# aligirayhanozbay/poisson_CNN

Measured on AMD Instinct MI355X. Metric: grids/sec (fwd+bwd) at 1024^2, higher is better.
Workload: dtype f32; 1 GPU; c4: Homogeneous_Poisson_NN_Legacy(hpnn.json) full train step (fwd+bwd+loss+Adam), 8 x 1024x1024 Dirichlet grids per GPU; global_batch=8, parallelism=dp1, math=fp32, ranks_seen=1

## Files before the change

include/pcnn.h:

```cpp
#ifndef PCNN_H
#define PCNN_H
#include <stddef.h>
#include <stdint.h>
#ifdef __cplusplus
extern "C" {
#endif

typedef struct pcnn_handle_s* pcnn_handle;

enum { PCNN_PAD_CONSTANT = 0, PCNN_PAD_SYMMETRIC = 1, PCNN_PAD_REFLECT = 2 };
enum { PCNN_ACT_LINEAR = 0, PCNN_ACT_LEAKY_RELU = 1, PCNN_ACT_TANH = 2, PCNN_ACT_RELU = 3 };
enum { PCNN_POOL_AVERAGE = 0, PCNN_POOL_MAX = 1 };
enum { PCNN_RESIZE_NEAREST = 0, PCNN_RESIZE_BILINEAR = 1, PCNN_RESIZE_BICUBIC = 2,
       PCNN_RESIZE_BICUBIC_LEGACY_ALIGN_CORNERS = 3  };

int pcnn_create(int device, void* hip_stream, pcnn_handle* out);
int pcnn_destroy(pcnn_handle h);
int pcnn_set_stream(pcnn_handle h, void* hip_stream);
int pcnn_sync(pcnn_handle h);
const char* pcnn_last_error(pcnn_handle h);
int pcnn_version(void);
uint32_t pcnn_crc32c(const void* data, size_t n, uint32_t crc);

#define PCNN_UNIQUE_ID_BYTES 128
// ... 52 lines not shown
                     const float* w1, const float* b1, const float* w2, const float* b2, float* o0, float* a1, float* o1, float* y);

int pcnn_conv2d_bwd_spectral_eligible(pcnn_handle h, const pcnn_conv_desc* d, const pcnn_conv_desc* dg);
int pcnn_conv2d_bwd_spectral(pcnn_handle h, const pcnn_conv_desc* d, const pcnn_conv_desc* dg, const float* x, const float* dz, const float* w_flipped,
                             const float* residual, float* dx, float* dw);
typedef struct pcnn_post_desc {
  const float* act_out; int ld_act_out; int act; float act_alpha;
  float* dbias; float* raw_out; int ld_raw;
} pcnn_post_desc;
int pcnn_conv2d_bwd_spectral_post_eligible(pcnn_handle h, const pcnn_conv_desc* d, const pcnn_conv_desc* dg);
int pcnn_conv2d_bwd_spectral_post(pcnn_handle h, const pcnn_conv_desc* d, const pcnn_conv_desc* dg, const float* x, const float* dz, const float* w_flipped,
                                  const float* residual, float* dx, float* dw, const pcnn_post_desc* post);

int pcnn_conv2d_dgrad_post_eligible(pcnn_handle h, const pcnn_conv_desc* dg, const float* dz, const float* residual, const float* dx, const pcnn_post_desc* post);
int pcnn_conv2d_dgrad_post(pcnn_handle h, const pcnn_conv_desc* dg, const float* dz, const float* w_flipped, const float* residual, float* dx,
                           const pcnn_post_desc* post);

int pcnn_debug_forward_spectrum32(pcnn_handle h, int H, int W, int C, const float* x, int Vy, int Vx, int oy, int ox, int pad_mode, float pad_value,
                                  int ylim, int xlim, int pack, float* out, size_t out_floats);
int pcnn_debug_tile_spectrum64(pcnn_handle h, int H, int W, int C, const float* x, int ylim, int xlim, float* out);

size_t pcnn_colsum_workspace(int C);
int pcnn_conv2d_epilogue_bwd(pcnn_handle h, int64_t npix, int C, const float* dy, int lddy, const float* a, int lda,
                             const float* bn_scale, int act, float act_alpha, float* dz, int lddz,
                             float* dbias, float* dsum_dy_a, float* dsum_dy, void* workspace, size_t workspace_bytes);
int pcnn_conv2d_epilogue_bwd_absmax(pcnn_handle h, int64_t npix, int C, const float* dy, int lddy, const float* a, int lda,
                                    const float* bn_scale, int act, float act_alpha, float* dz, int lddz, float* dbias,
                                    float* dsum_dy_a, float* dsum_dy, float* dz_absmax, void* workspace, size_t workspace_bytes);

int pcnn_pad_fold_bwd(pcnn_handle h, int N, int H, int W, int C, int pt, int pb, int pl, int pr, int pad_mode,
                      const float* gp, int ldgp, float* gx, int ldgx, int accumulate);
int pcnn_pad_fold_bwd_post_eligible(int C, int ldgp, int ld_add, const void* gp, const void* add_to, const pcnn_post_desc* post, int lddz, const void* dz);
int pcnn_pad_fold_bwd_post(pcnn_handle h, int N, int H, int W, int C, int pt, int pb, int pl, int pr, int pad_mode, const float* gp, int ldgp,
                           const float* add_to, int ld_add, const pcnn_post_desc* post, const float* bn_scale, float* dsum_dy_a, float* dsum_dy,
                           float* dz, int lddz, void* workspace, size_t workspace_bytes);

int pcnn_bn_fold(pcnn_handle h, int n, const float* gamma, const float* beta, const float* mean, const float* var, float eps,
                 float* scale, float* shift);
int pcnn_bn_fold_bwd(pcnn_handle h, int n, const float* s_dy_a, const float* s_dy, const float* mean, const float* var, float eps,
                     float* dgamma, float* dbeta);

int pcnn_channel_affine(pcnn_handle h, int64_t npix, int C, const float* x, int ldx, const float* scale, const float* shift,
                        const float* residual, int ld_res, float* y, int ldy);
int pcnn_bn_train_fwd(pcnn_handle h, int64_t npix, int C, const float* a, int lda, const float* gamma, const float* beta, float eps,
                      float momentum, float* moving_mean, float* moving_var, float* mean, float* inv_std, float* scale, float* scratch_2C,
                      const float* residual, int ld_res, float* y, int ldy, void* workspace, size_t workspace_bytes);
int pcnn_bn_train_bwd(pcnn_handle h, int64_t npix, int C, const float* dy, int lddy, const float* a, int lda, const float* scale,
                      const float* mean, const float* inv_std, float* dgamma, float* dbeta, float* scratch_4C, float* da, int ldda,
                      void* workspace, size_t workspace_bytes);

int pcnn_pool2d_fwd(pcnn_handle h, int kind, int N, int H, int W, int C, int f, const float* x, int ldx, float* y, int ldy);
int pcnn_pool2d_bwd(pcnn_handle h, int kind, int N, int H, int W, int C, int f, const float* x, int ldx,
                    const float* y, int ldy, const float* dy, int lddy, float* dx, int lddx, int accumulate);

int pcnn_deconv_fwd(pcnn_handle h, int N, int hc, int wc, int Cin, int H, int W, int Cout, int f, const float* x, int ldx,
                    const float* k, const float* bias, float alpha, float beta, float* y, int ldy);
int pcnn_deconv_bwd_data(pcnn_handle h, int N, int hc, int wc, int Cin, int H, int W, int Cout, int f, const float* dy, int lddy,
                         const float* k, float alpha, float* dx, int lddx);
size_t pcnn_deconv_wgrad_workspace(int N, int hc, int wc, int Cin, int Cout, int f);
int pcnn_deconv_bwd_filter(pcnn_handle h, int N, int hc, int wc, int Cin, int H, int W, int Cout, int f, const float* x, int ldx,
                           const float* dy, int lddy, float alpha, float* dk, float* dbias, void* workspace, size_t workspace_bytes);

typedef struct {
  int N, H, W, Cin, ldx;
  int Ho, Wo, Cout, ldy;
  int k;
  int act; float act_alpha;
  float dropout_rate; uint32_t dropout_seed; uint32_t dropout_layer;
  int ld_act_out;
  int accumulate;
} pcnn_wide_desc;
int pcnn_wide_conv2d_fwd(pcnn_handle h, const pcnn_wide_desc* d, const float* x, const float* w, const float* bias, float* y);
int pcnn_wide_conv2d_dgrad(pcnn_handle h, const pcnn_wide_desc* d, const float* dz, const float* wf, const float* act_out, float* dx);
size_t pcnn_wide_conv2d_wgrad_workspace(const pcnn_wide_desc* d);
int pcnn_wide_conv2d_wgrad(pcnn_handle h, const pcnn_wide_desc* d, const float* x, const float* dz, float* dw, float* dbias, void* workspace,
                           size_t workspace_bytes);
int pcnn_wide_deconv_fwd(pcnn_handle h, const pcnn_wide_desc* d, const float* x, const float* k, const float* bias, float* y);
int pcnn_wide_deconv_bwd_data(pcnn_handle h, const pcnn_wide_desc* d, const float* dz, const float* k, const float* act_out, float* dx);
size_t pcnn_wide_deconv_bwd_filter_workspace(const pcnn_wide_desc* d);
int pcnn_wide_deconv_bwd_filter(pcnn_handle h, const pcnn_wide_desc* d, const float* x, const float* dz, float* dk, void* workspace,
                                size_t workspace_bytes);

int pcnn_resize_tables(int method, int n_in, int n_out, int32_t* idx , float* wt );
int pcnn_resize_fwd(pcnn_handle h, int N, int hc, int wc, int C, int Ho, int Wo, const float* x, int ldx,
                    const int32_t* idx_y, const float* wt_y, const int32_t* idx_x, const float* wt_x,
                    float alpha, float beta, float* y, int ldy);
typedef struct pcnn_resize_src {
  const float* x; int hc, wc, ldx;
  const int32_t* idx_y; const float* wt_y; const int32_t* idx_x; const float* wt_x;
} pcnn_resize_src;
int pcnn_resize_fwd_multi_eligible(int N, int C, int Ho, int Wo, int nsrc, const pcnn_resize_src* src, const float* y, int ldy);
int pcnn_resize_fwd_multi(pcnn_handle h, int N, int C, int Ho, int Wo, int nsrc, const pcnn_resize_src* src, float alpha, float beta, float* y, int ldy);
int pcnn_resize_bwd(pcnn_handle h, int N, int hc, int wc, int C, int Ho, int Wo, const float* dy, int lddy,
                    const int32_t* idx_y, const float* wt_y, const int32_t* idx_x, const float* wt_x,
                    float alpha, float* tmp, float* dx, int lddx);

size_t pcnn_grouped_conv2d_wgrad_workspace(const pcnn_conv_desc* d);
int pcnn_grouped_conv2d_uses_mfma(const pcnn_conv_desc* d, int what);
int pcnn_grouped_conv2d_fwd(pcnn_handle h, const pcnn_conv_desc* d, const float* x, const float* w, long long w_sample_stride, const float* bias,
                            long long bias_sample_stride, int flip_transpose, float* y);
int pcnn_grouped_conv2d_wgrad(pcnn_handle h, const pcnn_conv_desc* d, const float* x, const float* dz, float* dw, long long dw_sample_stride, void* workspace);
int pcnn_grouped_bias_grad(pcnn_handle h, int N, long long HW, int C, const float* dz, int lddz, float* dbias, long long bias_sample_stride);
int pcnn_grouped_deconv_fwd(pcnn_handle h, int N, int H, int W, int Cin, int Ho, int Wo, int Cout, int f, const float* x, const float* k,
                            long long k_sample_stride, const float* bias, long long bias_sample_stride, float* y);
int pcnn_grouped_deconv_bwd_data(pcnn_handle h, int N, int H, int W, int Cin, int Ho, int Wo, int Cout, int f, const float* dy, const float* k,
                                 long long k_sample_stride, float* dx);
// ... 191 lines not shown
```

poisson_cnn_amd/csrc/pool_resize.hip:

```cpp
#include <math.h>
#include <vector>
#include "pcnn_internal.h"

namespace {

__device__ __forceinline__ void win(int o, int f, int pb, int n, int& a, int& b) {
  a = o * f - pb; b = a + f;
  if (a < 0) a = 0;
  if (b > n) b = n;
}

__global__ void pool_fwd_small_vec4_kernel(int kind, int N, int H, int W, int C, int f, int Ho, int Wo, int pby, int pbx,
                                           const float* __restrict__ x, int ldx, float* __restrict__ y, int ldy);
__global__ void pool_fwd_small_kernel(int kind, int N, int H, int W, int C, int f, int Ho, int Wo, int pby, int pbx,
                                      const float* __restrict__ x, int ldx, float* __restrict__ y, int ldy) {
  const int64_t total = (int64_t)N * Ho * Wo * C;
  for (int64_t i = (int64_t)blockIdx.x * blockDim.x + threadIdx.x; i < total; i += (int64_t)gridDim.x * blockDim.x) {
    const int c = i % C; int64_t r = i / C; const int ox = r % Wo; r /= Wo; const int oy = r % Ho; const int n = r / Ho;
    int y0, y1, x0, x1;
    win(oy, f, pby, H, y0, y1); win(ox, f, pbx, W, x0, x1);
    float acc = kind == PCNN_POOL_MAX ? -INFINITY : 0.f;
    for (int yy = y0; yy < y1; ++yy)
      for (int xx = x0; xx < x1; ++xx) {
        const float v = x[(((int64_t)n * H + yy) * W + xx) * ldx + c];
// ... 61 lines not shown
    int y0, y1, x0, x1;
    win(oy, f, pby, H, y0, y1); win(ox, f, pbx, W, x0, x1);
    const float cnt = (float)((y1 - y0) * (x1 - x0));
    const float* src = dy + (((int64_t)n * Ho + oy) * Wo + ox) * lddy + c;
    float* dst = dx + (((int64_t)n * H + yy) * W + xx) * lddx + c;
    if (V == 4) {
      const float4 g = *reinterpret_cast<const float4*>(src);
      float4 o = make_float4(g.x / cnt, g.y / cnt, g.z / cnt, g.w / cnt);
      if (accumulate) { const float4 d = *reinterpret_cast<const float4*>(dst); o.x += d.x; o.y += d.y; o.z += d.z; o.w += d.w; }
      *reinterpret_cast<float4*>(dst) = o;
    } else {
      const float g = *src / cnt;
      *dst = accumulate ? *dst + g : g;
    }
  }
}

__global__ void pool_bwd_max_kernel(int N, int H, int W, int C, int f, int Ho, int Wo, int pby, int pbx, const float* __restrict__ x, int ldx,
                                    const float* __restrict__ dy, int lddy, float* __restrict__ dx, int lddx) {
  const int64_t total = (int64_t)N * Ho * Wo * C;
  for (int64_t i = (int64_t)blockIdx.x * blockDim.x + threadIdx.x; i < total; i += (int64_t)gridDim.x * blockDim.x) {
    const int c = i % C; int64_t r = i / C; const int ox = r % Wo; r /= Wo; const int oy = r % Ho; const int n = r / Ho;
    int y0, y1, x0, x1;
    win(oy, f, pby, H, y0, y1); win(ox, f, pbx, W, x0, x1);
    float best = -INFINITY; int by = y0, bx = x0;
    for (int yy = y0; yy < y1; ++yy)
      for (int xx = x0; xx < x1; ++xx) {
        const float v = x[(((int64_t)n * H + yy) * W + xx) * ldx + c];
        if (v > best) { best = v; by = yy; bx = xx; }
      }
    dx[(((int64_t)n * H + by) * W + bx) * lddx + c] += dy[(((int64_t)n * Ho + oy) * Wo + ox) * lddy + c];
  }
}

__global__ void zero_strided_kernel(int64_t npix, int C, float* __restrict__ y, int ldy) {
  const int64_t total = npix * C;
  for (int64_t i = (int64_t)blockIdx.x * blockDim.x + threadIdx.x; i < total; i += (int64_t)gridDim.x * blockDim.x) y[(i / C) * ldy + i % C] = 0.f;
}

template <int V> struct ChanVec;
template <> struct ChanVec<1> {
  float v[1];
  __device__ static ChanVec load(const float* p) { ChanVec r; r.v[0] = *p; return r; }
  __device__ void store(float* p) const { *p = v[0]; }
};
template <> struct ChanVec<4> {
  float v[4];
  __device__ static ChanVec load(const float* p) {
    const float4 t = *reinterpret_cast<const float4*>(p);
    ChanVec r; r.v[0] = t.x; r.v[1] = t.y; r.v[2] = t.z; r.v[3] = t.w; return r;
  }
  __device__ void store(float* p) const { *reinterpret_cast<float4*>(p) = make_float4(v[0], v[1], v[2], v[3]); }
};

template <int V>
__global__ __launch_bounds__(256) void resize_fwd_kernel(int N, int hc, int wc, int C, int Ho, int Wo, const float* __restrict__ x, int ldx,
                                  const int32_t* __restrict__ iy, const float* __restrict__ wy, const int32_t* __restrict__ ix,
                                  const float* __restrict__ wx, float alpha, float beta, float* __restrict__ y, int ldy) {
  const int CV = C / V;
  const int64_t total = (int64_t)N * Ho * Wo * CV;
  for (int64_t i = (int64_t)blockIdx.x * blockDim.x + threadIdx.x; i < total; i += (int64_t)gridDim.x * blockDim.x) {
    const int c = (int)(i % CV) * V; int64_t r = i / CV; const int ox = r % Wo; r /= Wo; const int oy = r % Ho; const int n = r / Ho;
    float wxb[4]; int ixb[4];
#pragma unroll
    for (int b = 0; b < 4; ++b) { wxb[b] = wx[ox * 4 + b]; ixb[b] = ix[ox * 4 + b]; }
    float acc[V];
#pragma unroll
    for (int j = 0; j < V; ++j) acc[j] = 0.f;
#pragma unroll
    for (int a = 0; a < 4; ++a) {
      const float wya = wy[oy * 4 + a];
      if (wya == 0.f) continue;
      const float* row = x + ((int64_t)n * hc + iy[oy * 4 + a]) * wc * ldx + c;
      float t[V];
#pragma unroll
      for (int j = 0; j < V; ++j) t[j] = 0.f;
#pragma unroll
      for (int b = 0; b < 4; ++b) {
        if (wxb[b] != 0.f) {
          const ChanVec<V> q = ChanVec<V>::load(row + (int64_t)ixb[b] * ldx);
#pragma unroll
          for (int j = 0; j < V; ++j) t[j] += wxb[b] * q.v[j];
        }
      }
#pragma unroll
      for (int j = 0; j < V; ++j) acc[j] += wya * t[j];
    }
    float* dst = &y[(((int64_t)n * Ho + oy) * Wo + ox) * ldy + c];
    ChanVec<V> o;
    if (beta == 0.f) {
#pragma unroll
      for (int j = 0; j < V; ++j) o.v[j] = alpha * acc[j];
    } else {
      const ChanVec<V> old = ChanVec<V>::load(dst);
#pragma unroll
      for (int j = 0; j < V; ++j) o.v[j] = beta * old.v[j] + alpha * acc[j];
    }
    o.store(dst);
  }
}

constexpr int RESIZE_RPB = 8;
__global__ __launch_bounds__(256) void resize_fwd_y_kernel(int N, int hc, int C, int Ho, int Wo, const float* __restrict__ t, const int32_t* __restrict__ iy,
                                                           const float* __restrict__ wy, float alpha, float beta, float* __restrict__ y, int ldy) {
  const int CV = C >> 2;
  const int u = blockIdx.x * 256 + threadIdx.x;
// ... 201 lines not shown
}

static bool vec4_ok(int C, const void* a, int lda, const void* b, int ldb) {
  return C % 4 == 0 && lda % 4 == 0 && ldb % 4 == 0 && ((reinterpret_cast<uintptr_t>(a) | reinterpret_cast<uintptr_t>(b)) & 15) == 0;
}

static dim3 grid1d(int64_t total, int block = 256, int maxb = 16384) {
  int64_t b = pcnn_cdiv64(total, block);
  if (b > maxb) b = maxb;
  if (b < 1) b = 1;
  return dim3((unsigned)b);
}
static int pow2_ge(int c) { int p = 1; while (p < c) p <<= 1; return p; }

}

extern "C" int pcnn_pool2d_fwd(pcnn_handle h, int kind, int N, int H, int W, int C, int f, const float* x, int ldx, float* y, int ldy) {
  PCNN_REQUIRE(h, h && x && y && f >= 1 && (kind == 0 || kind == 1), "pcnn_pool2d_fwd: bad argument");
  const int Ho = pcnn_cdiv(H, f), Wo = pcnn_cdiv(W, f), pby = (Ho * f - H) / 2, pbx = (Wo * f - W) / 2;
  if (f * f <= 16 || C > 256) {
    if (vec4_ok(C, x, ldx, y, ldy))
      hipLaunchKernelGGL(pool_fwd_small_vec4_kernel, grid1d((int64_t)N * Ho * Wo * (C / 4)), dim3(256), 0, h->stream, kind, N, H, W, C, f, Ho, Wo, pby, pbx, x, ldx, y, ldy);
    else
      hipLaunchKernelGGL(pool_fwd_small_kernel, grid1d((int64_t)N * Ho * Wo * C), dim3(256), 0, h->stream, kind, N, H, W, C, f, Ho, Wo, pby, pbx, x, ldx, y, ldy);
  } else {
    hipLaunchKernelGGL(pool_fwd_large_kernel, dim3((unsigned)((int64_t)N * Ho * Wo)), dim3(256), 0, h->stream, kind, N, H, W, C, pow2_ge(C), f, Ho,
                       Wo, pby, pbx, x, ldx, y, ldy);
  }
  PCNN_CHECK_LAUNCH(h, "pcnn_pool2d_fwd");
  return 0;
}

extern "C" int pcnn_pool2d_bwd(pcnn_handle h, int kind, int N, int H, int W, int C, int f, const float* x, int ldx, const float* y, int ldy,
                               const float* dy, int lddy, float* dx, int lddx, int accumulate) {
  PCNN_REQUIRE(h, h && dy && dx && f >= 1 && (kind == 0 || kind == 1), "pcnn_pool2d_bwd: bad argument");
  (void)y; (void)ldy;
  const int Ho = pcnn_cdiv(H, f), Wo = pcnn_cdiv(W, f), pby = (Ho * f - H) / 2, pbx = (Wo * f - W) / 2;
  if (kind == PCNN_POOL_AVERAGE) {
    if (vec4_ok(C, dy, lddy, dx, lddx))
      hipLaunchKernelGGL(pool_bwd_avg_kernel<4>, grid1d((int64_t)N * H * W * (C / 4)), dim3(256), 0, h->stream, N, H, W, C, f, Ho, Wo, pby, pbx, dy, lddy, dx,
                         lddx, accumulate);
    else
      hipLaunchKernelGGL(pool_bwd_avg_kernel<1>, grid1d((int64_t)N * H * W * C), dim3(256), 0, h->stream, N, H, W, C, f, Ho, Wo, pby, pbx, dy, lddy, dx, lddx,
                         accumulate);
  } else {
    PCNN_REQUIRE(h, x, "pcnn_pool2d_bwd: max pooling needs the forward input");
    if (!accumulate) {
      hipLaunchKernelGGL(zero_strided_kernel, grid1d((int64_t)N * H * W * C), dim3(256), 0, h->stream, (int64_t)N * H * W, C, dx, lddx);
    }
    hipLaunchKernelGGL(pool_bwd_max_kernel, grid1d((int64_t)N * Ho * Wo * C), dim3(256), 0, h->stream, N, H, W, C, f, Ho, Wo, pby, pbx, x, ldx, dy, lddy, dx,
                       lddx);
  }
  PCNN_CHECK_LAUNCH(h, "pcnn_pool2d_bwd");
  return 0;
}

extern "C" int pcnn_resize_tables(int method, int n_in, int n_out, int32_t* idx, float* wt) {
  if (!idx || !wt || n_in < 1 || n_out < 1) return 1;
  const float scale = (float)n_in / (float)n_out;
  static std::vector<float> table;
  if (method == PCNN_RESIZE_BICUBIC && table.empty()) {
    const float a = -0.5f;
    table.resize((1024 + 1) * 2);
    for (int i = 0; i <= 1024; ++i) {
      float x = (float)i * 1.0f / 1024.0f;
      table[2 * i] = ((a + 2) * x - (a + 3)) * x * x + 1;
      x += 1.0f;
      table[2 * i + 1] = ((a * x - 5 * a) * x + 8 * a) * x - 4 * a;
    }
  }
  for (int o = 0; o < n_out; ++o) {
    int32_t* I = idx + 4 * o; float* Wt = wt + 4 * o;
    for (int k = 0; k < 4; ++k) { I[k] = 0; Wt[k] = 0.f; }
    if (method == PCNN_RESIZE_NEAREST) {
      int i = (int)floorf(((float)o + 0.5f) * scale);
      I[0] = i < 0 ? 0 : (i > n_in - 1 ? n_in - 1 : i); Wt[0] = 1.f;
    } else if (method == PCNN_RESIZE_BILINEAR) {
      const float src = ((float)o + 0.5f) * scale - 0.5f;
      const float fl = floorf(src);
      const int lo = fl > 0.f ? (int)fl : 0;
      const int hi = (int)fminf(ceilf(src), (float)(n_in - 1));
      const float lerp = src - fl;
      I[0] = lo; Wt[0] = 1.0f - lerp; I[1] = hi; Wt[1] = lerp;
    } else if (method == PCNN_RESIZE_BICUBIC) {
      const float src = ((float)o + 0.5f) * scale - 0.5f;
      const int loc = (int)floorf(src);
      const float delta = src - (float)loc;
      const int off = (int)lrintf(delta * 1024.0f);
      float w4[4] = {table[off * 2 + 1], table[off * 2], table[(1024 - off) * 2], table[(1024 - off) * 2 + 1]};
      float sum = 0.f;
      for (int k = 0; k < 4; ++k) {
        const int raw = loc - 1 + k;
        const int cl = raw < 0 ? 0 : (raw > n_in - 1 ? n_in - 1 : raw);
        if (cl != raw) w4[k] = 0.f;
        I[k] = cl; sum += w4[k];
      }
      if (fabsf(sum) >= 1000.0f * 1.17549435e-38f) {
        const float inv = 1.0f / sum;
        for (int k = 0; k < 4; ++k) w4[k] *= inv;
      }
      for (int k = 0; k < 4; ++k) Wt[k] = w4[k];
    } else if (method == PCNN_RESIZE_BICUBIC_LEGACY_ALIGN_CORNERS) {
      static std::vector<float> legacy;
      if (legacy.empty()) {
        const float a = -0.75f;
        legacy.resize((1024 + 1) * 2);
// ... 93 lines not shown
```

poisson_cnn_amd/models.py:

```python
import collections
import copy
import os

import numpy as np
import torch

from . import layers as L
from . import ops
from .utils import BC_EDGES, get_init_arguments_from_config, neumann_flags, neumann_mask, split_indices


def process_normalizations(normalizations):
    types, defaults = ['rhs_max_magnitude'], [False]
    if normalizations is None:
        return dict(zip(types, defaults))
    normalizations = dict(normalizations)
    for k, d in zip(types, defaults):
        normalizations.setdefault(k, d)
    if isinstance(normalizations['rhs_max_magnitude'], bool) and normalizations['rhs_max_magnitude']:
        normalizations['rhs_max_magnitude'] = 1.0
    return normalizations


def process_output_scaling_modes(output_scalings):
# ... 368 lines not shown
            history.update({'val_' + k: [] for k in self._VAL_KEYS})
        self.stop_training = False
        for cb in callbacks:
            cb.set_model(self)
        fetch = _Prefetcher(dataset, self.device)
        try:
            return self._fit_epochs(dataset, epochs, callbacks, verbose, steps_per_epoch, history, fetch, validation)
        finally:
            fetch.close()

    def _fit_epochs(self, dataset, epochs, callbacks, verbose, steps_per_epoch, history, fetch, validation=None):
        for epoch in range(epochs):
            n = steps_per_epoch if steps_per_epoch is not None else len(dataset)
            agg = {'loss': 0.0, 'mse': 0.0}
            logs = {'loss': float('nan'), 'mse': float('nan')}
            step = -1
            if n > 0:
                fetch.request(0)
            for step in range(n):
                inp, tar = fetch.take()
                logs = self.train_step((tuple(inp), tar))
                if step + 1 < n:
                    fetch.request(step + 1)
                logs = _host_logs(logs)
                for k in agg:
                    agg[k] += logs[k]
                for cb in callbacks:
                    cb.on_batch_end(step, logs)
                if self.stop_training:
                    break
            logs = {'loss': logs['loss'], 'mse': logs['mse'], 'lr': self.optimizer.learning_rate,
                    'loss_epoch_mean': agg['loss'] / max(step + 1, 1), 'mse_epoch_mean': agg['mse'] / max(step + 1, 1)}
            val_line = ''
            if validation is not None and (epoch + 1) % validation['freq'] == 0:
                res = self.evaluate(return_dict=True, **{k: v for k, v in validation.items() if k != 'freq'})
                logs.update({'val_' + k: res[k] for k in self._VAL_KEYS})
                val_line = ''.join(' - val_%s: %.6g' % (k, res[k]) for k in self._VAL_KEYS)
            for k in logs:
                history[k].append(logs[k])
            if verbose:
                print('Epoch %d/%d - loss: %.6g - mse: %.6g - lr: %.3g (epoch mean loss %.6g)%s'
                      % (epoch + 1, epochs, logs['loss'], logs['mse'], logs['lr'], logs['loss_epoch_mean'], val_line), flush=True)
            for cb in callbacks:
                cb.on_epoch_end(epoch, logs)
            if hasattr(dataset, 'on_epoch_end'):
                dataset.on_epoch_end()
            if self.stop_training:
                break
        return history


_BRANCH_STREAMS = os.environ.get('PCNN_BRANCH_STREAMS', '1') != '0'

MergePlan = collections.namedtuple('MergePlan', 'pyramid order stream tail')


def merge_plan(branches, H, W, coarse_factor):
    pyramid = {}
    for f in sorted({f for f, down, pool, _ in branches if down == 'pool' and pool in ('average', 'avg') and H % f == 0 and W % f == 0}):
        pyramid[f] = max([g for g in pyramid if f % g == 0], default=None)
    coarse = [i for i, b in enumerate(branches) if b[0] >= coarse_factor]
    order = [i for i in range(len(branches)) if i not in coarse] + coarse
    stream = {i: (k + 1 if branches[i][0] in pyramid else 0) for k, i in enumerate(coarse)}
    ntail = 0
    while ntail < min(3, len(order) - 1) and branches[order[-1 - ntail]][3] is not None:
        ntail += 1
    return MergePlan(pyramid, order, stream, order[len(order) - ntail:] if ntail >= 2 else [])


class _BottleneckMerge:

    def __init__(self, blocks, ctx, filters):
        self.blocks, self.ctx = list(blocks), ctx
        self.branches = [(b.f, b.down_method, b.pool, b.resize_method) for b in self.blocks]
        self.alpha = 1.0 / float(len(self.blocks) * filters)
        self._saved = None

    def pool_pyramid(self, x, plan):
        pyr = {}
        for f, parent in plan.pyramid.items():
            pyr[f] = ops.pool2d_fwd(x if parent is None else pyr[parent], f if parent is None else f // parent, 'average')
        return pyr

    def forward(self, initial, merged, training, coarse_factor):
        H, W = initial.shape[1], initial.shape[2]
        blocks, alpha = self.blocks, self.alpha
        plan = merge_plan(self.branches, H, W, coarse_factor)
        pyr = self.pool_pyramid(initial, plan)
        pending, streams = {}, {}
        if plan.stream and self.ctx.use_side and _BRANCH_STREAMS:
            ready = torch.cuda.Event()
            ready.record(torch.cuda.current_stream())
            for i, k in plan.stream.items():
                st = self.ctx.branch_stream(k)
                with torch.cuda.stream(st):
                    st.wait_event(ready)
                    o = blocks[i].forward_convs(initial, training, pyr.get(blocks[i].f))
                    done = torch.cuda.Event()
                    done.record(st)
                pending[i] = (o, done)
                if training:
                    streams[i] = st
        tail = []
        for n, i in enumerate(plan.order):
            b = blocks[i]
            if i in pending:
                o, done = pending[i]
                torch.cuda.current_stream().wait_event(done)
                o.record_stream(torch.cuda.current_stream())
            else:
                o = b.forward_convs(initial, training, pyr.get(b.f))
            b.note_upsampled(o, training)
            if i in plan.tail:
                tail.append((b, o))
            else:
                b.up_into(o, (H, W), merged, alpha, 0.0 if n == 0 else 1.0)
        if tail and ops.resize_fwd_multi([o for _, o in tail], (H, W), [b.resize_method for b, _ in tail], alpha=alpha, beta=1.0, out=merged) is None:
            for b, o in tail:
                b.up_into(o, (H, W), merged, alpha, 1.0)
        self._saved = (initial, pyr, plan.pyramid, streams) if training else None

    def backward(self, dmerged, d_initial):
        initial, pyr, parents, streams = self._saved
        self._saved = None
        alpha = self.alpha
        grads = {}
        late = []
        main = torch.cuda.current_stream()

        def add(f, g):
            grads[f] = g if f not in grads else ops.axpby(1.0, g, 1.0, grads[f])
        for i, b in enumerate(self.blocks):
            st = streams.get(i)
            if st is None:
                for _, g_prev, done_prev in late:
                    if g_prev is None:
                        main.wait_event(done_prev)
                g = b.backward_from(dmerged, alpha, d_initial)
                if g is not None:
                    add(b.f, g)
                continue
            dco = b.backward_up(dmerged, alpha)
            ev = torch.cuda.Event()
            ev.record(main)
            with torch.cuda.stream(st):
                st.wait_event(ev)
                dco.record_stream(st)
                g = b.backward_convs(dco, d_initial)
                done = torch.cuda.Event()
                done.record(st)
            late.append((b, g, done))
        for b, g, done in late:
            main.wait_event(done)
            if g is not None:
                g.record_stream(main)
                add(b.f, g)
        for f in sorted(grads, reverse=True):
            parent = parents[f]
            if parent is None:
                ops.pool2d_bwd(initial, grads[f], f, 'average', dx=d_initial, accumulate=True)
            else:
                if parent not in grads:
                    grads[parent] = torch.zeros_like(pyr[parent])
                ops.pool2d_bwd(pyr[parent], grads[f], f // parent, 'average', dx=grads[parent], accumulate=True)


class Homogeneous_Poisson_NN_Legacy(_ModelBase):
    model_name = 'Homogeneous_Poisson_NN_Legacy'

    def __init__(self, data_format='channels_first', final_convolutions_config=None, pre_bottleneck_convolutions_config=None,
                 bottleneck_deconv_config=None, bottleneck_multilinear_config=None, input_normalization=None, output_scaling=None,
                 use_batchnorm=False, postsmoother_iterations=5, use_scaling=False, use_positional_embeddings=True, scaling_config=None,
                 gradient_accumulation_steps=None, bc_type='dirichlet', device=None, seed=0, batchnorm_training=False, smoother_boundaries='frozen',
                 density_input=False, boundary_types=None):
        if data_format not in ('channels_first', 'channels_last'):
            raise ValueError('data_format must be channels_first or channels_last')
        if pre_bottleneck_convolutions_config is None:
            raise ValueError('Provide a config for pre bottleneck convolutions')
        if bottleneck_deconv_config is None or bottleneck_multilinear_config is None:
            raise ValueError('Provide a config for bottleneck blocks')
        if final_convolutions_config is None:
            raise ValueError('Provide a config for final convolutions')
        if bc_type is None:
            raise ValueError('bc_type can only be neumann or dirichlet.')
        flags = neumann_flags(bc_type)
        if smoother_boundaries not in ('frozen', 'enforce'):
            raise ValueError("smoother_boundaries can only be 'frozen' or 'enforce'.")
        self.density_input = bool(density_input)
        if self.density_input and (isinstance(bc_type, dict) or any(flags)):
            raise NotImplementedError('density_input=True needs bc_type "dirichlet": the variable-density solver, loss and smoother have Dirichlet edges '
                                      'only (got bc_type %r)' % (bc_type,))
        if boundary_types is not None:
            if not self.density_input:
                raise ValueError('boundary_types is the keyword of the variable-density model (density_input=True); the constant-coefficient '
                                 "model takes its boundary types as bc_type ('dirichlet', 'neumann' or a dict per edge), got boundary_types %r" % (boundary_types,))
            if not isinstance(boundary_types, dict):
                raise ValueError("boundary_types is None or a dict edge -> 'dirichlet' | 'neumann', got %r" % (boundary_types,))
            flags = neumann_flags(boundary_types)
        self.boundary_types = None if boundary_types is None else {e: 'neumann' if f else 'dirichlet' for e, f in zip(BC_EDGES, flags)}
        if self.density_input and data_format != 'channels_first':
            raise NotImplementedError('density_input=True: the two-channel stack is channels_first (N,2,H,W) only')
        self._init_device(device, _CPU_NOTE_RAISES)
        self.ndims = 2
        self.data_format = data_format
        self.gradient_accumulation_steps = gradient_accumulation_steps
        self.input_normalization = process_normalizations(input_normalization)
        self.output_scaling = process_output_scaling_modes(output_scaling)
        self.use_batchnorm = use_batchnorm
        self.use_positional_embeddings = use_positional_embeddings
        self.neumann_mask = neumann_mask(bc_type if boundary_types is None else boundary_types)
        self.per_edge_bc = isinstance(bc_type, dict)
        self.store = S = L.ParamStore()
        S.bn_training = bool(batchnorm_training)
        self.ctx = C = L.Context()
        C.enable_side_stream()

        pre = copy.deepcopy(pre_bottleneck_convolutions_config)
# ... 539 lines not shown
```

poisson_cnn_amd/ops.py:

```python
import ctypes
from ctypes import byref, c_float, c_int, c_int64, c_size_t, c_void_p

import numpy as np
import torch

from . import _lib
from ._lib import ConvDesc

PAD_MODES = {'CONSTANT': 0, 'SYMMETRIC': 1, 'REFLECT': 2}
ACTS = {'linear': 0, 'leaky_relu': 1, 'tanh': 2, 'relu': 3}
POOLS = {'average': 0, 'avg': 0, 'max': 1}
RESIZE = {'nearest': 0, 'bilinear': 1, 'bicubic': 2, 'bicubic_legacy': 3}
LEAKY_ALPHA = 0.2
BN_EPS = 1e-3

_handles = {}
MATH_MODES = {'fp32': 0, 'split_f16': 1}
_math_mode = MATH_MODES[__import__('os').environ.get('PCNN_MATH', 'fp32')]


def set_math_mode(mode):
    global _math_mode
    _math_mode = MATH_MODES[mode]
    for h in _handles.values():
# ... 486 lines not shown
    N, H, W, C = x.shape
    y = out if out is not None else empty((N, H, W, C), x.device)
    handle().call('pcnn_channel_affine', c_int64(N * H * W), c_int(C), _p(x), c_int(_ld(x)), _p(scale), _p(shift), _p(residual),
                  c_int(_ld(residual) if residual is not None else 0), _p(y), c_int(_ld(y)))
    return y


def bn_train_forward(a, gamma, beta, moving_mean, moving_var, residual=None, out=None, momentum=0.99, eps=BN_EPS, ws=None):
    N, H, W, C = a.shape
    lib = _lib.load()
    st = empty((5, C), a.device)
    mean, inv_std, scale = st[0], st[1], st[2]
    y = out if out is not None else empty((N, H, W, C), a.device)
    wsb = (ws or _default_ws).get(lib.pcnn_colsum_workspace(c_int(C)), a.device)
    handle().call('pcnn_bn_train_fwd', c_int64(N * H * W), c_int(C), _p(a), c_int(_ld(a)), _p(gamma), _p(beta), c_float(eps), c_float(momentum),
                  _p(moving_mean), _p(moving_var), _p(mean), _p(inv_std), _p(scale), _p(st[3:]), _p(residual),
                  c_int(_ld(residual) if residual is not None else 0), _p(y), c_int(_ld(y)), _p(wsb), c_size_t(wsb.numel() * 4))
    return y, (mean, inv_std, scale)


def bn_train_backward(dy, a, stats, dgamma, dbeta, ws=None):
    N, H, W, C = dy.shape
    mean, inv_std, scale = stats
    lib = _lib.load()
    tmp = empty((4, C), dy.device)
    wsb = (ws or _default_ws).get(lib.pcnn_colsum_workspace(c_int(C)), dy.device)
    da = empty((N, H, W, C), dy.device)
    handle().call('pcnn_bn_train_bwd', c_int64(N * H * W), c_int(C), _p(dy), c_int(_ld(dy)), _p(a), c_int(_ld(a)), _p(scale), _p(mean), _p(inv_std),
                  _p(dgamma), _p(dbeta), _p(tmp), _p(da), c_int(C), _p(wsb), c_size_t(wsb.numel() * 4))
    return da


def pool_out(n, f):
    return -(-n // f)


def pool2d_fwd(x, f, kind='average', out=None):
    N, H, W, C = x.shape
    y = out if out is not None else empty((N, pool_out(H, f), pool_out(W, f), C), x.device)
    handle().call('pcnn_pool2d_fwd', c_int(POOLS[kind.lower()]), c_int(N), c_int(H), c_int(W), c_int(C), c_int(f), _p(x), c_int(_ld(x)), _p(y), c_int(_ld(y)))
    return y


def pool2d_bwd(x, dy, f, kind='average', dx=None, accumulate=False):
    N, H, W, C = x.shape
    if dx is None:
        dx = empty((N, H, W, C), x.device)
        accumulate = False
    handle().call('pcnn_pool2d_bwd', c_int(POOLS[kind.lower()]), c_int(N), c_int(H), c_int(W), c_int(C), c_int(f), _p(x), c_int(_ld(x)),
                  c_void_p(0), c_int(0), _p(dy), c_int(_ld(dy)), _p(dx), c_int(_ld(dx)), c_int(1 if accumulate else 0))
    return dx


def _deconv_same_pads(k, hc, wc, H, W, f):
    kh, kw = k.shape[0], k.shape[1]
    if hc != -(-H // f) or wc != -(-W // f):
        raise ValueError('SAME transposed convolution needs input = ceil(output / stride): got %s for output %s at stride %d' % ((hc, wc), (H, W), f))
    return max((hc - 1) * f + kh - H, 0) // 2, max((wc - 1) * f + kw - W, 0) // 2


def _deconv_general_fwd(x, k, bias, out_hw, f, alpha, beta, out):
    N, hc, wc, Cin = x.shape
    kh, kw, Cout, _ = k.shape
    H, W = out_hw
    pt, pl = _deconv_same_pads(k, hc, wc, H, W, f)
    x_up = subsample_bwd(x, ((hc - 1) * f + 1, (wc - 1) * f + 1), f)
    y = conv2d_fwd(x_up, flip_transpose_weights(k.contiguous()), bias, pad_top=kh - 1 - pt, pad_left=kw - 1 - pl, out_hw=(H, W))
    if out is None:
        return y if alpha == 1.0 else axpby(alpha, y, 0.0, y)
    return axpby(alpha, y, beta, out)


def deconv_fwd(x, k, bias, out_hw, f, *, alpha=1.0, beta=0.0, out=None):
    N, hc, wc, Cin = x.shape
    Cout = k.shape[2]
    H, W = out_hw
    if k.shape[0] != f or k.shape[1] != f:
        return _deconv_general_fwd(x, k, bias, out_hw, f, alpha, beta, out)
    y = out if out is not None else empty((N, H, W, Cout), x.device)
    _launch('deconv_fwd', 2.0 * N * H * W * Cin * Cout,
            lambda: handle().call('pcnn_deconv_fwd', c_int(N), c_int(hc), c_int(wc), c_int(Cin), c_int(H), c_int(W), c_int(Cout), c_int(f), _p(x), c_int(_ld(x)),
                                  _p(k), _p(bias), c_float(alpha), c_float(beta), _p(y), c_int(_ld(y))),
            4.0 * (N * hc * wc * Cin + N * H * W * Cout * (2 if beta != 0.0 else 1) + f * f * Cin * Cout))
    return y


def deconv_bwd_data(dy, k, coarse_hw, f, *, alpha=1.0, out=None):
    N, H, W, Cout = dy.shape
    Cin = k.shape[3]
    hc, wc = coarse_hw
    if k.shape[0] != f or k.shape[1] != f:
        pt, pl = _deconv_same_pads(k, hc, wc, H, W, f)
        full = conv2d_fwd(dy, k.contiguous(), None, pad_top=pt, pad_left=pl, out_hw=((hc - 1) * f + 1, (wc - 1) * f + 1))
        dx_ = subsample(full, f)
        if alpha != 1.0:
            axpby(alpha, dx_, 0.0, dx_)
        if out is None:
            return dx_
        return axpby(1.0, dx_, 0.0, out)
    dx = out if out is not None else empty((N, hc, wc, Cin), dy.device)
    handle().call('pcnn_deconv_bwd_data', c_int(N), c_int(hc), c_int(wc), c_int(Cin), c_int(H), c_int(W), c_int(Cout), c_int(f), _p(dy), c_int(_ld(dy)),
                  _p(k), c_float(alpha), _p(dx), c_int(_ld(dx)))
    return dx


def deconv_bwd_filter(x, dy, f, *, alpha=1.0, dk=None, dbias=None, ws=None, kernel_size=None):
# ... 948 lines not shown
```

Measured before the change: 43.41 grids/s.

## Fuse multiple average-pool branches into single multi-factor pool kernels fwd and bwd

Adds multi-factor pooling kernels. The forward kernel tiles the input so that one block produces the pooled outputs for up to three factors, and the backward kernel sums the average-pool gradients from several factors into the input gradient in a single pass. The bottleneck merge now uses these for root pyramid levels and branch-owned pools. This reads the large input and read-modify-writes d_initial once instead of once per branch, at the cost of more complex tiling and fallback logic.

```diff
diff --git a/include/pcnn.h b/include/pcnn.h
--- a/include/pcnn.h
+++ b/include/pcnn.h
@@ -128,6 +128,10 @@
 int pcnn_pool2d_fwd(pcnn_handle h, int kind, int N, int H, int W, int C, int f, const float* x, int ldx, float* y, int ldy);
 int pcnn_pool2d_bwd(pcnn_handle h, int kind, int N, int H, int W, int C, int f, const float* x, int ldx,
                     const float* y, int ldy, const float* dy, int lddy, float* dx, int lddx, int accumulate);
+int pcnn_pool2d_fwd_multi(pcnn_handle h, int kind, int N, int H, int W, int C, int nf, const int* f, const float* x, int ldx, float* const* y,
+                          const int* ldy);
+int pcnn_pool2d_bwd_multi(pcnn_handle h, int kind, int N, int H, int W, int C, int nf, const int* f, const float* x, int ldx, const float* const* y,
+                          const int* ldy, const float* const* dy, const int* lddy, float* dx, int lddx, int accumulate);
 
 int pcnn_deconv_fwd(pcnn_handle h, int N, int hc, int wc, int Cin, int H, int W, int Cout, int f, const float* x, int ldx,
                     const float* k, const float* bias, float alpha, float beta, float* y, int ldy);
diff --git a/poisson_cnn_amd/csrc/pool_resize.hip b/poisson_cnn_amd/csrc/pool_resize.hip
--- a/poisson_cnn_amd/csrc/pool_resize.hip
+++ b/poisson_cnn_amd/csrc/pool_resize.hip
@@ -137,6 +137,74 @@
   }
   __device__ void store(float* p) const { *reinterpret_cast<float4*>(p) = make_float4(v[0], v[1], v[2], v[3]); }
 };
+
+struct PoolMultiFwd { int f[3], Ho[3], Wo[3], pby[3], pbx[3], ldy[3]; float* y[3]; };
+template <int V>
+__global__ __launch_bounds__(256) void pool_fwd_multi_kernel(int kind, int H, int W, int C, int nf, PoolMultiFwd a, int LY, int LX, int ty_org, int tx_org, int tiles_y,
+                                                             int tiles_x, const float* __restrict__ x, int ldx) {
+  const int CV = C / V;
+  int b = blockIdx.x;
+  const int tx = b % tiles_x; b /= tiles_x; const int ty = b % tiles_y; const int n = b / tiles_y;
+  const int ty0 = ty_org + ty * LY, tx0 = tx_org + tx * LX;
+  for (int k = 0; k < nf; ++k) {
+    const int f = a.f[k], Ho = a.Ho[k], Wo = a.Wo[k], pby = a.pby[k], pbx = a.pbx[k];
+    const int noy = LY / f, nox = LX / f;
+    const int oyb = (ty0 + pby) / f, oxb = (tx0 + pbx) / f;
+    const int items = noy * nox * CV;
+    for (int it = threadIdx.x; it < items; it += 256) {
+      const int c = (it % CV) * V; int r = it / CV; const int ox = oxb + r % nox, oy = oyb + r / nox;
+      if (oy < 0 || oy >= Ho || ox < 0 || ox >= Wo) continue;
+      int y0, y1, x0, x1;
+      win(oy, f, pby, H, y0, y1); win(ox, f, pbx, W, x0, x1);
+      const float init = kind == PCNN_POOL_MAX ? -INFINITY : 0.f;
+      ChanVec<V> acc;
+#pragma unroll
+      for (int j = 0; j < V; ++j) acc.v[j] = init;
+      for (int yy = y0; yy < y1; ++yy)
+        for (int xx = x0; xx < x1; ++xx) {
+          const ChanVec<V> v = ChanVec<V>::load(x + (((int64_t)n * H + yy) * W + xx) * ldx + c);
+#pragma unroll
+          for (int j = 0; j < V; ++j) acc.v[j] = kind == PCNN_POOL_MAX ? fmaxf(acc.v[j], v.v[j]) : acc.v[j] + v.v[j];
+        }
+      if (kind == PCNN_POOL_AVERAGE) {
+        const float d = (float)((y1 - y0) * (x1 - x0));
+#pragma unroll
+        for (int j = 0; j < V; ++j) acc.v[j] /= d;
+      }
+      acc.store(a.y[k] + (((int64_t)n * Ho + oy) * Wo + ox) * a.ldy[k] + c);
+    }
+  }
+}
+
+struct PoolMultiBwd { int f[3], Ho[3], Wo[3], pby[3], pbx[3], lddy[3]; const float* dy[3]; };
+template <int V, int NF>
+__global__ __launch_bounds__(256) void pool_bwd_avg_multi_kernel(int N, int H, int W, int C, PoolMultiBwd a, float* __restrict__ dx, int lddx, int accumulate) {
+  const int CV = C / V;
+  const int64_t total = (int64_t)N * H * W * CV;
+  for (int64_t i = (int64_t)blockIdx.x * blockDim.x + threadIdx.x; i < total; i += (int64_t)gridDim.x * blockDim.x) {
+    const int c = (int)(i % CV) * V; int64_t r = i / CV; const int xx = r % W; r /= W; const int yy = r % H; const int n = r / H;
+    float* dst = dx + (((int64_t)n * H + yy) * W + xx) * lddx + c;
+    ChanVec<V> g[NF], o;
+    float cnt[NF];
+#pragma unroll
+    for (int k = 0; k < NF; ++k) {
+      const int f = a.f[k], oy = (yy + a.pby[k]) / f, ox = (xx + a.pbx[k]) / f;
+      int y0, y1, x0, x1;
+      win(oy, f, a.pby[k], H, y0, y1); win(ox, f, a.pbx[k], W, x0, x1);
+      cnt[k] = (float)((y1 - y0) * (x1 - x0));
+      g[k] = ChanVec<V>::load(a.dy[k] + (((int64_t)n * a.Ho[k] + oy) * a.Wo[k] + ox) * a.lddy[k] + c);
+    }
+#pragma unroll
+    for (int j = 0; j < V; ++j) o.v[j] = 0.f;
+    if (accumulate) o = ChanVec<V>::load(dst);
+#pragma unroll
+    for (int k = 0; k < NF; ++k)
+#pragma unroll
+      for (int j = 0; j < V; ++j) o.v[j] = (k == 0 && !accumulate) ? g[k].v[j] / cnt[k] : g[k].v[j] / cnt[k] + o.v[j];
+    o.store(dst);
+  }
+}
+
 
 template <int V>
 __global__ __launch_bounds__(256) void resize_fwd_kernel(int N, int hc, int wc, int C, int Ho, int Wo, const float* __restrict__ x, int ldx,
@@ -444,6 +512,79 @@
                        lddx);
   }
   PCNN_CHECK_LAUNCH(h, "pcnn_pool2d_bwd");
+  return 0;
+}
+
+static bool pool_multi_origin(int nf, const int* f, const int* pb, int L, int* r_out) {
+  for (int r = 0; r < L; ++r) {
+    bool ok = true;
+    for (int k = 0; k < nf; ++k) ok = ok && r % f[k] == pb[k] % f[k];
+    if (ok) { *r_out = r; return true; }
+  }
+  return false;
+}
+
+extern "C" int pcnn_pool2d_fwd_multi(pcnn_handle h, int kind, int N, int H, int W, int C, int nf, const int* f, const float* x, int ldx, float* const* y,
+                                     const int* ldy) {
+  PCNN_REQUIRE(h, h && x && y && f && ldy && nf >= 1 && nf <= 3 && (kind == 0 || kind == 1), "pcnn_pool2d_fwd_multi: bad argument");
+  for (int k = 0; k < nf; ++k) PCNN_REQUIRE(h, f[k] >= 1 && y[k], "pcnn_pool2d_fwd_multi: bad argument");
+  PoolMultiFwd a = {};
+  int fs[3], pby[3], pbx[3], m = 0, L = 1;
+  bool vec = C % 4 == 0 && ldx % 4 == 0 && (reinterpret_cast<uintptr_t>(x) & 15) == 0, fused[3] = {false, false, false};
+  for (int k = 0; k < nf; ++k) {
+    if (!(f[k] * f[k] <= 16 || C > 256)) continue;
+    const int Ho = pcnn_cdiv(H, f[k]), Wo = pcnn_cdiv(W, f[k]);
+    fs[m] = a.f[m] = f[k]; a.Ho[m] = Ho; a.Wo[m] = Wo; pby[m] = a.pby[m] = (Ho * f[k] - H) / 2; pbx[m] = a.pbx[m] = (Wo * f[k] - W) / 2;
+    a.y[m] = y[k]; a.ldy[m] = ldy[k];
+    vec = vec && ldy[k] % 4 == 0 && (reinterpret_cast<uintptr_t>(y[k]) & 15) == 0;
+    int g = L, t = f[k];
+    while (t) { const int q = g % t; g = t; t = q; }
+    L = L <= 48 ? L / g * f[k] : L;
+    fused[k] = true; ++m;
+  }
+  int ry = 0, rx = 0;
+  if (m >= 2 && L <= 48 && pool_multi_origin(m, fs, pby, L, &ry) && pool_multi_origin(m, fs, pbx, L, &rx)) {
+    const int LY = L, LX = L * (96 / L);
+    const int tiles_y = pcnn_cdiv(H + ry, LY), tiles_x = pcnn_cdiv(W + rx, LX);
+    const int64_t blocks = (int64_t)N * tiles_y * tiles_x;
+    if (blocks < ((int64_t)1 << 31)) {
+      if (vec) hipLaunchKernelGGL(pool_fwd_multi_kernel<4>, dim3((unsigned)blocks), dim3(256), 0, h->stream, kind, H, W, C, m, a, LY, LX, -ry, -rx, tiles_y, tiles_x, x, ldx);
+      else hipLaunchKernelGGL(pool_fwd_multi_kernel<1>, dim3((unsigned)blocks), dim3(256), 0, h->stream, kind, H, W, C, m, a, LY, LX, -ry, -rx, tiles_y, tiles_x, x, ldx);
+      PCNN_CHECK_LAUNCH(h, "pcnn_pool2d_fwd_multi");
+    } else {
+      m = 0;
+    }
+  } else {
+    m = 0;
+  }
+  for (int k = 0; k < nf; ++k)
+    if (!(m && fused[k]) && pcnn_pool2d_fwd(h, kind, N, H, W, C, f[k], x, ldx, y[k], ldy[k])) return 1;
+  return 0;
+}
+
+extern "C" int pcnn_pool2d_bwd_multi(pcnn_handle h, int kind, int N, int H, int W, int C, int nf, const int* f, const float* x, int ldx, const float* const* y,
+                                     const int* ldy, const float* const* dy, const int* lddy, float* dx, int lddx, int accumulate) {
+  PCNN_REQUIRE(h, h && dy && lddy && dx && f && nf >= 1 && nf <= 3 && (kind == 0 || kind == 1), "pcnn_pool2d_bwd_multi: bad argument");
+  for (int k = 0; k < nf; ++k) PCNN_REQUIRE(h, f[k] >= 1 && dy[k], "pcnn_pool2d_bwd_multi: bad argument");
+  if (kind != PCNN_POOL_AVERAGE || nf == 1) {
+    for (int k = 0; k < nf; ++k)
+      if (pcnn_pool2d_bwd(h, kind, N, H, W, C, f[k], x, ldx, y ? y[k] : nullptr, ldy ? ldy[k] : 0, dy[k], lddy[k], dx, lddx, k ? 1 : accumulate)) return 1;
+    return 0;
+  }
+  PoolMultiBwd a = {};
+  bool vec = C % 4 == 0 && lddx % 4 == 0 && (reinterpret_cast<uintptr_t>(dx) & 15) == 0;
+  for (int k = 0; k < nf; ++k) {
+    a.f[k] = f[k]; a.Ho[k] = pcnn_cdiv(H, f[k]); a.Wo[k] = pcnn_cdiv(W, f[k]);
+    a.pby[k] = (a.Ho[k] * f[k] - H) / 2; a.pbx[k] = (a.Wo[k] * f[k] - W) / 2;
+    a.dy[k] = dy[k]; a.lddy[k] = lddy[k];
+    vec = vec && lddy[k] % 4 == 0 && (reinterpret_cast<uintptr_t>(dy[k]) & 15) == 0;
+  }
+  const dim3 grid = grid1d((int64_t)N * H * W * (vec ? C / 4 : C));
+  if (vec && nf == 2) hipLaunchKernelGGL((pool_bwd_avg_multi_kernel<4, 2>), grid, dim3(256), 0, h->stream, N, H, W, C, a, dx, lddx, accumulate);
+  else if (vec) hipLaunchKernelGGL((pool_bwd_avg_multi_kernel<4, 3>), grid, dim3(256), 0, h->stream, N, H, W, C, a, dx, lddx, accumulate);
+  else if (nf == 2) hipLaunchKernelGGL((pool_bwd_avg_multi_kernel<1, 2>), grid, dim3(256), 0, h->stream, N, H, W, C, a, dx, lddx, accumulate);
+  else hipLaunchKernelGGL((pool_bwd_avg_multi_kernel<1, 3>), grid, dim3(256), 0, h->stream, N, H, W, C, a, dx, lddx, accumulate);
+  PCNN_CHECK_LAUNCH(h, "pcnn_pool2d_bwd_multi");
   return 0;
 }
 
diff --git a/poisson_cnn_amd/models.py b/poisson_cnn_amd/models.py
--- a/poisson_cnn_amd/models.py
+++ b/poisson_cnn_amd/models.py
@@ -444,10 +444,10 @@
 
 _BRANCH_STREAMS = os.environ.get('PCNN_BRANCH_STREAMS', '1') != '0'
 
-MergePlan = collections.namedtuple('MergePlan', 'pyramid order stream tail')
-
-
-def merge_plan(branches, H, W, coarse_factor):
+MergePlan = collections.namedtuple('MergePlan', 'pyramid order stream tail fused', defaults=((),))
+
+
+def merge_plan(branches, H, W, coarse_factor, fuse_pools=True):
     pyramid = {}
     for f in sorted({f for f, down, pool, _ in branches if down == 'pool' and pool in ('average', 'avg') and H % f == 0 and W % f == 0}):
         pyramid[f] = max([g for g in pyramid if f % g == 0], default=None)
@@ -457,7 +457,13 @@
     ntail = 0
     while ntail < min(3, len(order) - 1) and branches[order[-1 - ntail]][3] is not None:
         ntail += 1
-    return MergePlan(pyramid, order, stream, order[len(order) - ntail:] if ntail >= 2 else [])
+    fused = ()
+    if fuse_pools and all(down == 'pool' and pool in ('average', 'avg') for _, down, pool, _ in branches):
+        own = [b[0] for b in branches if b[0] not in pyramid]
+        roots = sorted((f for f, parent in pyramid.items() if parent is None), reverse=True)
+        if len(set(own)) == len(own) and len(own) + len(roots) >= 2:
+            fused = tuple(own + roots)
+    return MergePlan(pyramid, order, stream, order[len(order) - ntail:] if ntail >= 2 else [], fused)
 
 
 class _BottleneckMerge:
@@ -468,16 +474,22 @@
         self.alpha = 1.0 / float(len(self.blocks) * filters)
         self._saved = None
 
+    fuse_pools = True
+
     def pool_pyramid(self, x, plan):
         pyr = {}
+        first = sorted(plan.fused)
+        for k in range(0, len(first), 3):
+            pyr.update(zip(first[k:k + 3], ops.pool2d_fwd_multi(x, first[k:k + 3], 'average')))
         for f, parent in plan.pyramid.items():
-            pyr[f] = ops.pool2d_fwd(x if parent is None else pyr[parent], f if parent is None else f // parent, 'average')
+            if f not in pyr:
+                pyr[f] = ops.pool2d_fwd(x if parent is None else pyr[parent], f if parent is None else f // parent, 'average')
         return pyr
 
     def forward(self, initial, merged, training, coarse_factor):
         H, W = initial.shape[1], initial.shape[2]
         blocks, alpha = self.blocks, self.alpha
-        plan = merge_plan(self.branches, H, W, coarse_factor)
+        plan = merge_plan(self.branches, H, W, coarse_factor, self.fuse_pools)
         pyr = self.pool_pyramid(initial, plan)
         pending, streams = {}, {}
         if plan.stream and self.ctx.use_side and _BRANCH_STREAMS:
@@ -510,10 +522,10 @@
         if tail and ops.resize_fwd_multi([o for _, o in tail], (H, W), [b.resize_method for b, _ in tail], alpha=alpha, beta=1.0, out=merged) is None:
             for b, o in tail:
                 b.up_into(o, (H, W), merged, alpha, 1.0)
-        self._saved = (initial, pyr, plan.pyramid, streams) if training else None
+        self._saved = (initial, pyr, plan.pyramid, streams, plan.fused) if training else None
 
     def backward(self, dmerged, d_initial):
-        initial, pyr, parents, streams = self._saved
+        initial, pyr, parents, streams, fused = self._saved
         self._saved = None
         alpha = self.alpha
         grads = {}
@@ -548,13 +560,17 @@
                 g.record_stream(main)
                 add(b.f, g)
         for f in sorted(grads, reverse=True):
-            parent = parents[f]
+            parent = parents.get(f)
+            if f in fused:
+                continue
             if parent is None:
                 ops.pool2d_bwd(initial, grads[f], f, 'average', dx=d_initial, accumulate=True)
             else:
                 if parent not in grads:
                     grads[parent] = torch.zeros_like(pyr[parent])
                 ops.pool2d_bwd(pyr[parent], grads[f], f // parent, 'average', dx=grads[parent], accumulate=True)
+        for k in range(0, len(fused), 3):
+            ops.pool2d_bwd_multi(initial, [grads[f] for f in fused[k:k + 3]], fused[k:k + 3], 'average', dx=d_initial, accumulate=True)
 
 
 class Homogeneous_Poisson_NN_Legacy(_ModelBase):
diff --git a/poisson_cnn_amd/ops.py b/poisson_cnn_amd/ops.py
--- a/poisson_cnn_amd/ops.py
+++ b/poisson_cnn_amd/ops.py
@@ -562,6 +562,27 @@
     return dx
 
 
+def pool2d_fwd_multi(x, factors, kind='average'):
+    N, H, W, C = x.shape
+    nf = len(factors)
+    ys = [empty((N, pool_out(H, f), pool_out(W, f), C), x.device) for f in factors]
+    handle().call('pcnn_pool2d_fwd_multi', c_int(POOLS[kind.lower()]), c_int(N), c_int(H), c_int(W), c_int(C), c_int(nf), (c_int * nf)(*factors), _p(x), c_int(_ld(x)),
+                  (c_void_p * nf)(*[y.data_ptr() for y in ys]), (c_int * nf)(*[_ld(y) for y in ys]))
+    return ys
+
+
+def pool2d_bwd_multi(x, dys, factors, kind='average', dx=None, accumulate=False):
+    N, H, W, C = x.shape
+    nf = len(factors)
+    if dx is None:
+        dx = empty((N, H, W, C), x.device)
+        accumulate = False
+    handle().call('pcnn_pool2d_bwd_multi', c_int(POOLS[kind.lower()]), c_int(N), c_int(H), c_int(W), c_int(C), c_int(nf), (c_int * nf)(*factors), _p(x), c_int(_ld(x)),
+                  c_void_p(0), c_void_p(0), (c_void_p * nf)(*[d.data_ptr() for d in dys]), (c_int * nf)(*[_ld(d) for d in dys]), _p(dx), c_int(_ld(dx)),
+                  c_int(1 if accumulate else 0))
+    return dx
+
+
 def _deconv_same_pads(k, hc, wc, H, W, f):
     kh, kw = k.shape[0], k.shape[1]
     if hc != -(-H // f) or wc != -(-W // f):
```

Measured after the change: 43.58 grids/s (median of 6 runs). Within noise of the previous version (+0.4%).
